# Foxhead-Studio/InsTaG

Measured on AMD Instinct MI355X. Metric: train-step frames/sec @512x512, 100k Gaussians, higher is better.
Workload: dtype f32; 1 GPU; C3: train_face step, 100k Gaussians + 6 grid encodes + UMF/PMF motion nets (DeepSpeech feats), 512x512, SH degree 1, image + attention map in one raster pass, L1+DSSIM, Adam; targets = uniform noise (SURVEY 8d); gaussians=100000, sh_degree=1, parallelism=dp1, ranks_reported_by_backend=1, execution=hipGraph replay, timing=one window of 1714 steps after 5 warm-up steps

## Files before the change

### instag_amd/csrc/common.hpp

```cpp
#pragma once
#include <hip/hip_runtime.h>
#include <stdint.h>
#include <stddef.h>
#include <algorithm>
#include <mutex>
#include <set>
#include <string>
#include <utility>

#include "instag_hip.h"

namespace instag {

void set_error(const std::string& msg);

#define INSTAG_CHECK_HIP(expr)                                                                  \
  do {                                                                                          \
    hipError_t _e = (expr);                                                                     \
    if (_e != hipSuccess) {                                                                     \
      ::instag::set_error(std::string(#expr) + ": " + hipGetErrorString(_e));                   \
      return INSTAG_E_HIP;                                                                      \
    }                                                                                           \
  } while (0)

#define INSTAG_REQUIRE(cond, msg)                                                               \
  do {                                                                                          \
    if (!(cond)) {                                                                              \
      ::instag::set_error(std::string(msg));                                                    \
      return INSTAG_E_ARG;                                                                      \
    }                                                                                           \
  } while (0)

#define INSTAG_CHECK_LAUNCH() INSTAG_CHECK_HIP(hipGetLastError())

#define INSTAG_TRY(expr) do { if (int rc_ = (expr)) return rc_; } while (0)

enum ProfKernel {
  K_PREPROCESS = 0, K_DUPLICATE = 1, K_SORT = 2, K_RANGES = 3, K_BLEND_FWD = 4, K_BLEND_BWD = 5,
  K_PREPROCESS_BWD = 6, K_GRID_FWD = 7, K_GRID_BWD = 8, K_SH_FWD = 9, K_SH_BWD = 10,
  K_MLP_FWD = 11, K_MLP_BWD = 12, K_MLP_WGRAD = 13, K_LOSS_FWD = 14, K_LOSS_BWD = 15, K_BLEND_BWD_MEAN = 16,
  K_EMPTY_BRACKET = 17,
};
struct ProfScope {
  ProfScope(int kernel, hipStream_t stream);
  ~ProfScope();
  int kernel_;
  hipStream_t stream_;
  hipEvent_t start_ = nullptr;
  int graph_slot_ = -1;
};

template <typename T>
static inline T div_up(T a, T b) { return (a + b - 1) / b; }

static inline int set_max_dynamic_lds(const void* kernel, int bytes) {
  static std::mutex mu;
  static std::set<std::pair<const void*, int>> done;
  int dev = 0;
  INSTAG_CHECK_HIP(hipGetDevice(&dev));
  std::lock_guard<std::mutex> lk(mu);
  if (done.count({kernel, dev})) return INSTAG_OK;
  INSTAG_CHECK_HIP(hipFuncSetAttribute(kernel, hipFuncAttributeMaxDynamicSharedMemorySize, bytes));
  done.insert({kernel, dev});
  return INSTAG_OK;
}

static inline size_t align_up(size_t v, size_t a) { return (v + a - 1) / a * a; }

struct Arena {
  size_t off = 0;
  size_t take(size_t n) { const size_t o = off; off += align_up(n, 64); return o; }
};

constexpr int TILE_X = 16;
constexpr int TILE_Y = 16;
constexpr int REC_FLOATS = 16;

enum RecSlot { R_X = 0, R_Y, R_CA, R_CB, R_CC, R_OP, R_R, R_G, R_B, R_DEPTH, R_NX, R_NY, R_NZ, R_EXTRA,
               R_OFFSET, R_RECT };

struct GeomLayout {
  size_t rec2d, cov3d, tiles_touched, point_offsets, flags, cull_thr;
  size_t depth_key, depth_key_alt, order_a, order;
  size_t dsort_zero, dsort_zero_words;
  size_t dsort_digit_base;
  size_t dsort_partials;
  size_t scan_state, scan_state_words;
  size_t tile_partials, tile_total, tile_dropped, pre_zero_words;
  uint32_t pre_blocks;
  uint32_t dsort_blocks, dkey_blocks;
  size_t total;
};
GeomLayout geom_layout(int32_t N);

struct ImageLayout {
  size_t ranges, n_contrib, final_T;
  size_t tile_rounds;
  size_t blend_mode;
  size_t total;
};
ImageLayout image_layout(int32_t H, int32_t W);

struct BinningLayout {
  size_t keys_unsorted, vals_unsorted, keys, vals, ktmp, vtmp, gid_unsorted, point_list;
  size_t tsort_zero, tsort_zero_words;
  size_t tsort_digit_base;
  size_t tsort_partials;
  size_t sort_count;
  uint32_t tsort_blocks;
  size_t seg_state, seg_slots, seg_queue, seg_count, row_flag, row_flag_stride;
  size_t fwd_sync, seg_flag;
  size_t total;
};
constexpr int SEG_LEN = 128;
constexpr int SEG_FLOATS = 14;
constexpr int TILE_PIX = TILE_X * TILE_Y;
BinningLayout binning_layout(int64_t R, int32_t H, int32_t W);

}
```

### instag_amd/csrc/grid.hip

```cpp
#include <cstdlib>

#include "common.hpp"
#include "device_math.hpp"

namespace instag {
namespace {

constexpr int GRID_BLOCK = 256;
constexpr uint32_t LDS_BUDGET_FLOATS = 16384;

template <uint32_t D>
__device__ __forceinline__ uint32_t fast_hash(const uint32_t pos_grid[D]) {
  constexpr uint32_t primes[7] = {1u, 2654435761u, 805459861u, 3674653429u, 2097192037u, 1434869437u, 2165219737u};
  uint32_t result = 0;
#pragma unroll
  for (uint32_t i = 0; i < D; ++i) result ^= pos_grid[i] * primes[i];
  return result;
}

template <uint32_t D>
__device__ __forceinline__ uint32_t grid_index(uint32_t gridtype, bool align_corners, uint32_t hashmap_size,
                                               uint32_t resolution, const uint32_t pos_grid[D]) {
  uint32_t stride = 1, index = 0;
#pragma unroll
// ... 453 lines not shown

inline bool dc_supported(uint32_t D, uint32_t C) { return D >= 2 && D <= 5 && (C == 1 || C == 2 || C == 4 || C == 8); }

#define DISPATCH_DC(D, C, FN, ...)                                                            \
  switch (D) {                                                                                \
    case 2: switch (C) { case 1: return FN<2, 1>(__VA_ARGS__); case 2: return FN<2, 2>(__VA_ARGS__); \
                         case 4: return FN<2, 4>(__VA_ARGS__); case 8: return FN<2, 8>(__VA_ARGS__); } break; \
    case 3: switch (C) { case 1: return FN<3, 1>(__VA_ARGS__); case 2: return FN<3, 2>(__VA_ARGS__); \
                         case 4: return FN<3, 4>(__VA_ARGS__); case 8: return FN<3, 8>(__VA_ARGS__); } break; \
    case 4: switch (C) { case 1: return FN<4, 1>(__VA_ARGS__); case 2: return FN<4, 2>(__VA_ARGS__); \
                         case 4: return FN<4, 4>(__VA_ARGS__); case 8: return FN<4, 8>(__VA_ARGS__); } break; \
    case 5: switch (C) { case 1: return FN<5, 1>(__VA_ARGS__); case 2: return FN<5, 2>(__VA_ARGS__); \
                         case 4: return FN<5, 4>(__VA_ARGS__); case 8: return FN<5, 8>(__VA_ARGS__); } break; \
  }

}
}

using namespace instag;

extern "C" {

int instag_grid_encode_forward(const float* inputs, const float* embeddings, const int32_t* offsets, float* outputs,
                               uint32_t B, uint32_t D, uint32_t C, uint32_t L, float S, uint32_t H, float* dy_dx,
                               uint32_t gridtype, int align_corners, uint32_t interp, instag_stream_t stream) {
  INSTAG_REQUIRE(L >= 1 && L <= 64, "GridEncoding: L must be in [1,64]");
  INSTAG_REQUIRE(dc_supported(D, C), "GridEncoding: D must be 2..5 and C must be 1, 2, 4, or 8.");
  if (B == 0) return INSTAG_OK;
  INSTAG_REQUIRE(inputs && embeddings && offsets && outputs, "grid_encode_forward: NULL tensor");
  hipStream_t s = (hipStream_t)stream;
  DISPATCH_DC(D, C, run_forward, inputs, embeddings, offsets, outputs, B, L, S, H, dy_dx, gridtype,
              align_corners != 0, interp, s);
  set_error("GridEncoding: D must be 2..5 and C must be 1, 2, 4, or 8.");
  return INSTAG_E_ARG;
}

int instag_grid_encode_backward(const float* grad, const float* inputs, const float* embeddings,
                                const int32_t* offsets, float* grad_embeddings, uint32_t B, uint32_t D, uint32_t C,
                                uint32_t L, float S, uint32_t H, const float* dy_dx, float* grad_inputs,
                                uint32_t gridtype, int align_corners, uint32_t interp, instag_stream_t stream) {
  (void)embeddings;
  INSTAG_REQUIRE(L >= 1 && L <= 64, "GridEncoding: L must be in [1,64]");
  INSTAG_REQUIRE(dc_supported(D, C), "GridEncoding: D must be 2..5 and C must be 1, 2, 4, or 8.");
  if (B == 0) return INSTAG_OK;
  INSTAG_REQUIRE(grad && inputs && offsets && grad_embeddings, "grid_encode_backward: NULL tensor");
  hipStream_t s = (hipStream_t)stream;
  DISPATCH_DC(D, C, run_backward, grad, inputs, offsets, grad_embeddings, B, L, S, H, dy_dx, grad_inputs,
              gridtype, align_corners != 0, interp, s);
  set_error("GridEncoding: D must be 2..5 and C must be 1, 2, 4, or 8.");
  return INSTAG_E_ARG;
}

size_t instag_grid_total_variation_workspace_bytes(uint32_t total_params, uint32_t C) {
  return align_up((size_t)total_params * sizeof(uint32_t), 256) + (size_t)total_params * C * sizeof(unsigned long long);
}

int instag_grid_total_variation(const float* inputs, const float* embeddings, float* grad, const int32_t* offsets,
                                float weight, uint32_t B, uint32_t D, uint32_t C, uint32_t L, float S, uint32_t H,
                                uint32_t gridtype, int align_corners, uint32_t total_params, void* workspace,
                                size_t workspace_bytes, instag_stream_t stream) {
  INSTAG_REQUIRE(L >= 1 && L <= 64, "GridEncoding: L must be in [1,64]");
  INSTAG_REQUIRE(dc_supported(D, C), "GridEncoding: D must be 2..5 and C must be 1, 2, 4, or 8.");
  if (B == 0) return INSTAG_OK;
  INSTAG_REQUIRE(inputs && embeddings && grad && offsets, "grad_total_variation: NULL tensor");
  const size_t need = instag_grid_total_variation_workspace_bytes(total_params, C);
  if (workspace == nullptr || workspace_bytes < need) { set_error("grad_total_variation: workspace too small"); return INSTAG_E_SPACE; }
  hipStream_t s = (hipStream_t)stream;
  INSTAG_CHECK_HIP(hipMemsetAsync(workspace, 0, need, s));
  uint32_t* counts = (uint32_t*)workspace;
  unsigned long long* acc = (unsigned long long*)((char*)workspace + align_up((size_t)total_params * sizeof(uint32_t), 256));
  DISPATCH_DC(D, C, run_tv, inputs, embeddings, grad, offsets, weight, B, L, S, H, gridtype, align_corners != 0, counts,
              acc, s);
  set_error("GridEncoding: D must be 2..5 and C must be 1, 2, 4, or 8.");
  return INSTAG_E_ARG;
}

}

namespace instag {
namespace {

constexpr uint32_t TP_MAX_L = 16;
inline bool tp_fits_lds(uint32_t total_params) { return (size_t)12 * total_params <= 156 * 1024; }

struct TriPlaneArgs {
  const float* xyz;
  const float* tables[3];
  const int32_t* offsets;
  uint32_t N, L, H;
  float S, bound;
  const float* shift;
  uint32_t shift_stride;
  float shift_scale;
};

__device__ __forceinline__ void tp_point(const TriPlaneArgs& a, uint32_t b, float p[3]) {
#pragma unroll
  for (int k = 0; k < 3; ++k) p[k] = a.xyz[3 * b + k];
  if (a.shift) {
#pragma unroll
    for (int k = 0; k < 3; ++k) p[k] += a.shift_scale * a.shift[(size_t)b * a.shift_stride + k];
  }
}

__device__ __forceinline__ void plane_coords(int plane, const float p[3], float x[2]) {
  x[0] = plane == 1 ? p[1] : p[0];
  x[1] = plane == 0 ? p[1] : p[2];
}

struct TpLevel { float scale; uint32_t stride, offset; };

__device__ __forceinline__ void tp_levels(const TriPlaneArgs& a, TpLevel* s_lv) {
  if (threadIdx.x < a.L) {
    const LevelGeom lg = level_geom(a.offsets, threadIdx.x, a.S, a.H);
    s_lv[threadIdx.x] = TpLevel{lg.scale, lg.resolution + 1, (uint32_t)a.offsets[threadIdx.x]};
  }
}

template <int THREADS, bool ZERO_ACC>
__device__ __forceinline__ void tp_stage_table(float* __restrict__ s_tab, float* __restrict__ s_acc,
                                               const float* __restrict__ tab, uint32_t T) {
  if ((T & 3u) == 0 && (reinterpret_cast<uintptr_t>(tab) & 15) == 0) {
    const float4* src = reinterpret_cast<const float4*>(tab);
    float4* dst = reinterpret_cast<float4*>(s_tab);
    float4* acc = reinterpret_cast<float4*>(s_acc);
    const uint32_t n4 = T >> 2;
#pragma unroll 8
    for (uint32_t i = threadIdx.x; i < n4; i += THREADS) {
      dst[i] = src[i];
      if (ZERO_ACC) acc[i] = make_float4(0.f, 0.f, 0.f, 0.f);
    }
  } else {
#pragma unroll 8
    for (uint32_t i = threadIdx.x; i < T; i += THREADS) {
      s_tab[i] = tab[i];
      if (ZERO_ACC) s_acc[i] = 0.f;
    }
  }
}

__global__ void __launch_bounds__(GRID_BLOCK)
triplane_forward_kernel(TriPlaneArgs a, float* __restrict__ out ) {
  extern __shared__ __align__(16) float s_tab[];
  __shared__ TpLevel s_lv[TP_MAX_L];
  const uint32_t per_block = (a.N + gridDim.x - 1) / gridDim.x;
  const uint32_t b0 = blockIdx.x * per_block, b1 = min(a.N, b0 + per_block);
  const uint32_t T = (uint32_t)a.offsets[a.L];
  const float inv2b = 1.0f / (2.0f * a.bound);
  tp_levels(a, s_lv);
  for (int plane = 0; plane < 3; ++plane) {
    __syncthreads();
    tp_stage_table<GRID_BLOCK, false>(s_tab, nullptr, a.tables[plane], T);
    __syncthreads();
    for (uint32_t b = b0 + threadIdx.x; b < b1; b += GRID_BLOCK) {
      float p[3];
      tp_point(a, b, p);
      float xw[2];
      plane_coords(plane, p, xw);
      const float x0 = (xw[0] + a.bound) * inv2b, x1 = (xw[1] + a.bound) * inv2b;
      const bool oob = x0 < 0.f || x0 > 1.f || x1 < 0.f || x1 > 1.f;
      float* o = out + (size_t)b * 3 * a.L + plane * a.L;
#pragma unroll 4
      for (uint32_t l = 0; l < a.L; ++l) {
        float v = 0.f;
        if (!oob) {
          const TpLevel lv = s_lv[l];
// ... 637 lines not shown
```

### instag_amd/csrc/mlp.hip

```cpp
#include <cstdlib>

#include "common.hpp"

namespace instag {
namespace {

using f32x16 = __attribute__((ext_vector_type(16))) float;
constexpr int MLP_BLOCK = 256;

__device__ __forceinline__ constexpr int feat(int r, int h) { return (r & 3) + 8 * (r >> 2) + 4 * h; }

template <int KC = 0>
__device__ __forceinline__ void load_block(const float* __restrict__ X, size_t row, bool valid, int Krt, int b, int h,
                                           f32x16& v) {
  const int K = KC > 0 ? KC : Krt;
  const float* __restrict__ base = X + (valid ? row * (size_t)K : 0);
  if ((K & 3) == 0) {
#pragma unroll
    for (int q = 0; q < 4; ++q) {
      const int f0 = 32 * b + 8 * q + 4 * h;
      const bool ok = valid && f0 < K;
      const float4 t = *reinterpret_cast<const float4*>(base + (ok ? f0 : 0));
      v[4 * q + 0] = ok ? t.x : 0.f; v[4 * q + 1] = ok ? t.y : 0.f;
      v[4 * q + 2] = ok ? t.z : 0.f; v[4 * q + 3] = ok ? t.w : 0.f;
// ... 239 lines not shown
            }
          }
          raw[b][4 * q] = t.x; raw[b][4 * q + 1] = t.y; raw[b][4 * q + 2] = t.z; raw[b][4 * q + 3] = t.w;
        }
    } else {
#pragma unroll
      for (int b = 0; b < KB0; ++b) load_block(X, row, valid, d.K0, b, h, raw[b]);
    }
  };
  int tile = blockIdx.x * 4 + wave;
  if (tile < ntiles) fetch(tile);
  for (; tile < ntiles; tile += tstride) {
    const size_t row = (size_t)tile * 32 + l31;
    const bool valid = row < (size_t)d.N;
    f32x16 in0[KB0];
#pragma unroll
    for (int b = 0; b < KB0; ++b) in0[b] = raw[b];
    if (tile + tstride < ntiles) fetch(tile + tstride);
    if (GLUE) {
      constexpr int K0 = GLUE_KX + GLUE_KA + GLUE_KE;
      float sa = 0.f, se = 0.f;
#pragma unroll
      for (int b = 0; b < KB0; ++b)
#pragma unroll
        for (int q = 0; q < 4; ++q) {
          const int f0 = 32 * b + 8 * q + 4 * h;
          float v[4] = {in0[b][4 * q], in0[b][4 * q + 1], in0[b][4 * q + 2], in0[b][4 * q + 3]};
          if (f0 >= GLUE_KX && f0 + 4 <= GLUE_KX + GLUE_KA) {
            sa += (v[0] * v[0] + v[1] * v[1]) + (v[2] * v[2] + v[3] * v[3]);
#pragma unroll
            for (int i = 0; i < 4; ++i) v[i] *= mul[b][4 * q + i];
          } else if (f0 >= GLUE_KX + GLUE_KA && f0 < K0) {
#pragma unroll
            for (int i = 0; i < 4; ++i)
              if (f0 + i < K0) {
                const float act = fmaxf(v[i], 0.f);
                se += act * act;
                v[i] = mul[b][4 * q + i] * act;
              }
          }
          if (valid && f0 < K0 && gf.h_in != nullptr) {
            float* hp = gf.h_in + row * K0 + f0;
            *reinterpret_cast<float2*>(hp) = make_float2(v[0], v[1]);
            if (f0 + 2 < K0) *reinterpret_cast<float2*>(hp + 2) = make_float2(v[2], v[3]);
          }
          in0[b][4 * q] = v[0]; in0[b][4 * q + 1] = v[1]; in0[b][4 * q + 2] = v[2]; in0[b][4 * q + 3] = v[3];
        }
      sa += __shfl_xor(sa, 32);
      se += __shfl_xor(se, 32);
      if (valid && h == 0) { gf.amb[3 * row] = sqrtf(sa); gf.amb[3 * row + 1] = sqrtf(se); gf.amb[3 * row + 2] = 0.f; }
    }
    f32x16 h1[HB];
    layer_forward<KQ0, KB0, HB>(w1, in0, h1, l31, h);
    relu_blocks<HB>(h1);
    if (A1) {
      store_blocks<HB, 8 * HQ>(A1, row, valid, d.H, h, h1);
    }
    f32x16 out[1];
    if (NL == 3) {
      f32x16 h2[HB];
      uint32_t sw1 = 0, sw2 = 0;
      layer_forward<HQ, HB, HB, KEEP>(w2, h1, h2, l31, h, &sw1);
      if constexpr (KEEP) S1[(size_t)tile * 64 + lane] = sw1;
      relu_blocks<HB>(h2);
      if (A2) {
        store_blocks<HB, 8 * HQ>(A2, row, valid, d.H, h, h2);
      }
      layer_forward<HQ, HB, 1, KEEP>(w3, h2, out, l31, h, &sw2);
      if constexpr (KEEP) S2[(size_t)tile * 64 + lane] = sw2;
    } else {
      uint32_t sw1 = 0;
      layer_forward<HQ, HB, 1, KEEP>(w2, h1, out, l31, h, &sw1);
      if constexpr (KEEP) S1[(size_t)tile * 64 + lane] = sw1;
    }
    store_block(Y, row, valid, d.O, 0, h, out[0]);
  }
}

struct GlueBwd {
  const float* aud; const float* eye_pre; const float* enc_a; const float* enc_e; const float* amb; const float* d_amb;
  float* d_enc_x; float* d_aud; float* d_eye; float* col_partials;
};

template <int KQ0, int HQ, int OQ, int NL, bool GLUE = false>
__global__ void __launch_bounds__(MLP_BLOCK) __attribute__((amdgpu_waves_per_eu(2)))
mlp_backward_kernel(MlpDims d, const float* __restrict__ dY, const uint32_t* __restrict__ S1,
                    const uint32_t* __restrict__ S2, const float* __restrict__ W1, const float* __restrict__ W2,
                    const float* __restrict__ W3, float* __restrict__ dZ1, float* __restrict__ dZ2,
                    float* dX, const float* dXadd ,
                    GlueBwd gl = GlueBwd{}) {
  extern __shared__ __align__(16) float s_w[];
  __shared__ float s_col[GLUE ? 4 : 1][GLUE ? 40 : 1];
  constexpr int KBG = (KQ0 + 3) / 4;
  float part[GLUE ? KBG : 1][4][4];
  if (GLUE) {
#pragma unroll
    for (int b = 0; b < KBG; ++b)
#pragma unroll
      for (int q = 0; q < 4; ++q)
#pragma unroll
        for (int i = 0; i < 4; ++i) part[b][q][i] = 0.f;
  }
  constexpr int KB0 = (KQ0 + 3) / 4, HB = (HQ + 3) / 4;
  constexpr int KP0 = KB0 * 32, HP = HB * 32;
  float* w1 = s_w;
  float* w2 = w1 + HP * (KP0 + 1);
  float* w3 = w2 + (NL == 3 ? HP : 32) * (HP + 1);
  if (dX || GLUE) stage_weights<HP, KB0>(w1, W1, d.H, d.K0);
  stage_weights<(NL == 3 ? HP : 32), HB>(w2, W2, NL == 3 ? d.H : d.O, d.H);
  if (NL == 3) stage_weights<32, HB>(w3, W3, d.O, d.H);
  __syncthreads();
  const int lane = threadIdx.x & 63, wave = threadIdx.x >> 6, l31 = lane & 31, h = lane >> 5;
  const int ntiles = (d.N + 31) / 32;
  const int tstride = gridDim.x * 4;
  f32x16 ndy;
  uint32_t ns1 = 0, ns2 = 0;
  auto fetch = [&](int tile) {
    const size_t row = (size_t)tile * 32 + l31;
    const bool valid = row < (size_t)d.N;
    load_block(dY, row, valid, d.O, 0, h, ndy);
    if constexpr (NL == 3) ns2 = S2[(size_t)tile * 64 + lane];
    ns1 = S1[(size_t)tile * 64 + lane];
  };
  int tile = blockIdx.x * 4 + wave;
  if (tile < ntiles) fetch(tile);
  for (; tile < ntiles; tile += tstride) {
    const size_t row = (size_t)tile * 32 + l31;
    const bool valid = row < (size_t)d.N;
    f32x16 dy[1];
    dy[0] = ndy;
    const uint32_t s1 = ns1, s2 = ns2;
    if (tile + tstride < ntiles) fetch(tile + tstride);
    f32x16 g1[HB];
    if constexpr (NL == 3) {
      f32x16 g2[HB];
      layer_backward<OQ, 1, HB>(w3, dy, g2, l31, h);
      mask_blocks<HB>(g2, s2);
      store_blocks<HB, 8 * HQ>(dZ2, row, valid, d.H, h, g2);
      layer_backward<HQ, HB, HB>(w2, g2, g1, l31, h);
    } else {
      layer_backward<OQ, 1, HB>(w2, dy, g1, l31, h);
    }
    mask_blocks<HB>(g1, s1);
    store_blocks<HB, 8 * HQ>(dZ1, row, valid, d.H, h, g1);
    if (GLUE) {
      f32x16 gx[KB0];
      layer_backward<HQ, HB, KB0>(w1, g1, gx, l31, h);
      if (valid) {
        const float na = gl.amb[3 * row], ne = gl.amb[3 * row + 1];
        const float ga = (gl.d_amb && na > 0.f) ? gl.d_amb[3 * row] / na : 0.f;
        const float ge = (gl.d_amb && ne > 0.f) ? gl.d_amb[3 * row + 1] / ne : 0.f;
#pragma unroll
        for (int b = 0; b < KB0; ++b)
#pragma unroll
          for (int q = 0; q < 4; ++q) {
            const int f0 = 32 * b + 8 * q + 4 * h;
            const float gw[4] = {gx[b][4 * q], gx[b][4 * q + 1], gx[b][4 * q + 2], gx[b][4 * q + 3]};
            if (f0 + 4 <= GLUE_KX) {
              *reinterpret_cast<float4*>(gl.d_enc_x + row * GLUE_KX + f0) = make_float4(gw[0], gw[1], gw[2], gw[3]);
            } else if (f0 >= GLUE_KX && f0 + 4 <= GLUE_KX + GLUE_KA) {
              const int k = f0 - GLUE_KX;
              const float4 a = *reinterpret_cast<const float4*>(gl.aud + row * GLUE_KA + k);
              const float4 ea = *reinterpret_cast<const float4*>(gl.enc_a + k);
              *reinterpret_cast<float4*>(gl.d_aud + row * GLUE_KA + k) =
                  make_float4(ea.x * gw[0] + ga * a.x, ea.y * gw[1] + ga * a.y, ea.z * gw[2] + ga * a.z,
                              ea.w * gw[3] + ga * a.w);
              part[b][q][0] += gw[0] * a.x; part[b][q][1] += gw[1] * a.y;
              part[b][q][2] += gw[2] * a.z; part[b][q][3] += gw[3] * a.w;
            } else if (f0 >= GLUE_KX + GLUE_KA && f0 < GLUE_KX + GLUE_KA + GLUE_KE) {
              const int k = f0 - GLUE_KX - GLUE_KA;
#pragma unroll
              for (int i = 0; i < 4; ++i) {
                if (k + i < GLUE_KE) {
                  const float pre = gl.eye_pre[row * GLUE_KE + k + i];
                  const float act = fmaxf(pre, 0.f);
                  gl.d_eye[row * GLUE_KE + k + i] = pre > 0.f ? (gl.enc_e[k + i] * gw[i] + ge * act) : 0.f;
                  part[b][q][i] += gw[i] * act;
                }
              }
            }
          }
      }
    } else if (dX) {
      f32x16 gx[KB0];
      layer_backward<HQ, HB, KB0>(w1, g1, gx, l31, h);
      if (dXadd) {
#pragma unroll
        for (int b = 0; b < KB0; ++b) {
          f32x16 prev;
          load_block(dXadd, row, valid, d.K0, b, h, prev);
          gx[b] += prev;
        }
      }
#pragma unroll
      for (int b = 0; b < KB0; ++b) store_block(dX, row, valid, d.K0, b, h, gx[b]);
    }
  }
  if (GLUE) {
    for (int i = threadIdx.x; i < 4 * 40; i += MLP_BLOCK) (&s_col[0][0])[i] = 0.f;
    __syncthreads();
#pragma unroll
    for (int b = 0; b < KBG; ++b)
#pragma unroll
      for (int q = 0; q < 4; ++q) {
        const int f0 = 32 * b + 8 * q + 4 * h;
        if (f0 >= GLUE_KX && f0 < GLUE_KX + GLUE_KA + GLUE_KE) {
#pragma unroll
          for (int i = 0; i < 4; ++i) {
            float v = part[b][q][i];
#pragma unroll
            for (int o = 16; o > 0; o >>= 1) v += __shfl_xor(v, o);
            if (l31 == 0 && f0 + i < GLUE_KX + GLUE_KA + GLUE_KE) s_col[wave][f0 + i - GLUE_KX] = v;
          }
        }
      }
    __syncthreads();
    if ((int)threadIdx.x < GLUE_KA + GLUE_KE)
      gl.col_partials[(size_t)blockIdx.x * (GLUE_KA + GLUE_KE) + threadIdx.x] =
          ((s_col[0][threadIdx.x] + s_col[1][threadIdx.x]) + s_col[2][threadIdx.x]) + s_col[3][threadIdx.x];
  }
}


struct Mlp2Dims { int N, K0, HA, OA, HB, OB; };

template <int KQ0, int HQA, int HQB>
size_t mlp2_lds_bytes() {
  constexpr int KP0 = (KQ0 + 3) / 4 * 32, HPA = (HQA + 3) / 4 * 32, HPB = (HQB + 3) / 4 * 32;
  return sizeof(float) * (HPA * (KP0 + 1) + 32 * (HPA + 1) + HPB * (KP0 + 1) + 32 * (HPB + 1));
}

template <int KQ0, int HQA, int OQA, int HQB, int OQB, bool KEEP >
__global__ void __launch_bounds__(MLP_BLOCK)
mlp2_forward_kernel(Mlp2Dims d, const float* __restrict__ X, const float* __restrict__ WA1,
                    const float* __restrict__ WA2, const float* __restrict__ WB1, const float* __restrict__ WB2,
                    float* __restrict__ YA, float* __restrict__ YB, float* __restrict__ A1A, float* __restrict__ A1B,
                    uint32_t* __restrict__ S1) {
  extern __shared__ __align__(16) float s_w[];
  constexpr int KB0 = (KQ0 + 3) / 4, HBA = (HQA + 3) / 4, HBB = (HQB + 3) / 4;
  constexpr int KP0 = KB0 * 32, HPA = HBA * 32, HPB = HBB * 32;
  static_assert(HBA == 1 && HBB == 1, "mlp2: the two heads' sign bits share one word per lane");
  float* wa1 = s_w;
  float* wa2 = wa1 + HPA * (KP0 + 1);
  float* wb1 = wa2 + 32 * (HPA + 1);
  float* wb2 = wb1 + HPB * (KP0 + 1);
  stage_weights<HPA, KB0>(wa1, WA1, d.HA, d.K0);
  stage_weights<32, HBA>(wa2, WA2, d.OA, d.HA);
  stage_weights<HPB, KB0>(wb1, WB1, d.HB, d.K0);
  stage_weights<32, HBB>(wb2, WB2, d.OB, d.HB);
  __syncthreads();
  const int lane = threadIdx.x & 63, wave = threadIdx.x >> 6, l31 = lane & 31, h = lane >> 5;
  const int ntiles = (d.N + 31) / 32;
  for (int tile = blockIdx.x * 4 + wave; tile < ntiles; tile += gridDim.x * 4) {
    const size_t row = (size_t)tile * 32 + l31;
    const bool valid = row < (size_t)d.N;
    f32x16 in0[KB0];
#pragma unroll
    for (int b = 0; b < KB0; ++b) load_block(X, row, valid, d.K0, b, h, in0[b]);
    uint32_t sw = 0;
    {
      f32x16 h1[HBA], out[1];
      layer_forward<KQ0, KB0, HBA>(wa1, in0, h1, l31, h);
      relu_blocks<HBA>(h1);
      if (A1A) store_blocks<HBA, 8 * HQA>(A1A, row, valid, d.HA, h, h1);
      layer_forward<HQA, HBA, 1, KEEP>(wa2, h1, out, l31, h, &sw);
      store_block(YA, row, valid, d.OA, 0, h, out[0]);
    }
    {
      f32x16 h1[HBB], out[1];
      layer_forward<KQ0, KB0, HBB>(wb1, in0, h1, l31, h);
      relu_blocks<HBB>(h1);
      if (A1B) store_blocks<HBB, 8 * HQB>(A1B, row, valid, d.HB, h, h1);
      layer_forward<HQB, HBB, 1, KEEP, 16>(wb2, h1, out, l31, h, &sw);
      store_block(YB, row, valid, d.OB, 0, h, out[0]);
    }
    if constexpr (KEEP) S1[(size_t)tile * 64 + lane] = sw;
  }
}

template <int KQ0, int HQA, int OQA, int HQB, int OQB>
__global__ void __launch_bounds__(MLP_BLOCK)
mlp2_backward_kernel(Mlp2Dims d, const float* __restrict__ dYA, const float* __restrict__ dYB,
                     const uint32_t* S1A, const uint32_t* S1B , const float* __restrict__ WA1,
                     const float* __restrict__ WA2, const float* __restrict__ WB1, const float* __restrict__ WB2,
                     float* __restrict__ dZ1A, float* __restrict__ dZ1B, float* dX,
                     const float* dXadd ) {
  extern __shared__ __align__(16) float s_w[];
  constexpr int KB0 = (KQ0 + 3) / 4, HBA = (HQA + 3) / 4, HBB = (HQB + 3) / 4;
  constexpr int KP0 = KB0 * 32, HPA = HBA * 32, HPB = HBB * 32;
  static_assert(HBA == 1 && HBB == 1, "mlp2: the two heads' sign bits share one word per lane");
  float* wa1 = s_w;
  float* wa2 = wa1 + HPA * (KP0 + 1);
  float* wb1 = wa2 + 32 * (HPA + 1);
  float* wb2 = wb1 + HPB * (KP0 + 1);
  if (dX) { stage_weights<HPA, KB0>(wa1, WA1, d.HA, d.K0); stage_weights<HPB, KB0>(wb1, WB1, d.HB, d.K0); }
  stage_weights<32, HBA>(wa2, WA2, d.OA, d.HA);
  stage_weights<32, HBB>(wb2, WB2, d.OB, d.HB);
  __syncthreads();
  const int lane = threadIdx.x & 63, wave = threadIdx.x >> 6, l31 = lane & 31, h = lane >> 5;
  const int ntiles = (d.N + 31) / 32;
  const int tstride = gridDim.x * 4;
  f32x16 ndya, ndyb;
  uint32_t nsa = 0, nsb = 0;
// ... 29 lines not shown
    }
    {
      f32x16 g1[HBB], gb[KB0];
      layer_backward<OQB, 1, HBB>(wb2, dyb, g1, l31, h);
      mask_blocks<HBB, 16>(g1, sb);
      store_blocks<HBB, 8 * HQB>(dZ1B, row, valid, d.HB, h, g1);
      if (dX) {
        layer_backward<HQB, HBB, KB0>(wb1, g1, gb, l31, h);
#pragma unroll
        for (int b = 0; b < KB0; ++b) gx[b] += gb[b];
      }
    }
    if (dX) {
      if (dXadd) {
#pragma unroll
        for (int b = 0; b < KB0; ++b) {
          f32x16 prev;
          load_block(dXadd, row, valid, d.K0, b, h, prev);
          gx[b] += prev;
        }
      }
#pragma unroll
      for (int b = 0; b < KB0; ++b) store_block(dX, row, valid, d.K0, b, h, gx[b]);
    }
  }
}

struct WgVirt {
  int job;
  const float *xb, *xc, *mb, *mc;
  int Ka, Kb, Kc, pad;
};

template <int OB, int KB, bool VIRT = false>
__device__ __forceinline__ void weight_grad_body(const float* __restrict__ dZ, const float* __restrict__ In, int N, int O,
                                                 int K, float* __restrict__ partial, float* s_acc, int block,
                                                 int nblocks, const WgVirt* virt = nullptr) {
  constexpr int TILES = OB * KB;
  constexpr int TW = TILES >= 4 ? 4 : TILES;
  constexpr int RS = 4 / TW;
  constexpr int MYT = (TILES + TW - 1) / TW;
  const int lane = threadIdx.x & 63, wave = threadIdx.x >> 6, l31 = lane & 31, h = lane >> 5;
  const int tw = wave % TW, rs = wave / TW;
  const bool busy = wave < TW * RS;
  const int per_block = (((N + nblocks - 1) / nblocks) + 1) & ~1;
  const long b0 = (long)block * per_block, b1 = min((long)N, b0 + per_block);
  const int per_split = ((((int)max(0l, b1 - b0) + RS - 1) / RS) + 1) & ~1;
  const long w0 = b0 + (long)rs * per_split;
  const long w1 = busy ? min(b1, w0 + per_split) : w0;
  int tt[MYT], tb[MYT];
  bool live[MYT], oin[MYT], kin[MYT];
#pragma unroll
  for (int j = 0; j < MYT; ++j) {
    const int idx = tw + j * TW;
    live[j] = idx < TILES;
    tt[j] = live[j] ? idx / KB : 0;
    tb[j] = live[j] ? idx % KB : 0;
    oin[j] = live[j] && 32 * tt[j] + l31 < O;
    kin[j] = live[j] && 32 * tb[j] + l31 < K;
  }
  const float* bp[MYT];
  int bs[MYT];
  float bm[MYT];
  bool brelu[MYT];
#pragma unroll
  for (int j = 0; j < MYT; ++j) {
    const int col = 32 * tb[j] + l31;
    bp[j] = In + col; bs[j] = K; bm[j] = 1.f; brelu[j] = false;
    if (VIRT && kin[j]) {
      if (col < virt->Ka) { bp[j] = In + col; bs[j] = virt->Ka; }
      else if (col < virt->Ka + virt->Kb) {
        bp[j] = virt->xb + (col - virt->Ka); bs[j] = virt->Kb; bm[j] = virt->mb[col - virt->Ka];
      } else {
        const int c2 = col - virt->Ka - virt->Kb;
        bp[j] = virt->xc + c2; bs[j] = virt->Kc; bm[j] = virt->mc[c2]; brelu[j] = true;
      }
    }
  }
  f32x16 acc[MYT];
#pragma unroll
  for (int j = 0; j < MYT; ++j)
#pragma unroll
    for (int i = 0; i < 16; ++i) acc[j][i] = 0.f;
  constexpr int UNROLL = 6;
  for (long r0 = w0; r0 < w1; r0 += 2 * UNROLL) {
    float a[UNROLL][MYT], bb[UNROLL][MYT];
#pragma unroll
    for (int u = 0; u < UNROLL; ++u) {
      const long row = r0 + 2 * u + h;
      const bool ok = row < w1;
#pragma unroll
      for (int j = 0; j < MYT; ++j) {
        a[u][j] = (ok && oin[j]) ? dZ[row * O + 32 * tt[j] + l31] : 0.f;
        float v = (ok && kin[j]) ? bp[j][row * bs[j]] : 0.f;
        if (VIRT) {
          v = brelu[j] ? fmaxf(v, 0.f) : v;
          v *= bm[j];
        }
        bb[u][j] = v;
      }
    }
#pragma unroll
    for (int u = 0; u < UNROLL; ++u)
#pragma unroll
      for (int j = 0; j < MYT; ++j)
        acc[j] = __builtin_amdgcn_mfma_f32_32x32x2f32(a[u][j], bb[u][j], acc[j], 0, 0, 0);
  }
  float* dst = partial + (size_t)block * O * K;
  if (RS == 1) {
#pragma unroll
    for (int j = 0; j < MYT; ++j) {
      if (!live[j] || !busy) continue;
#pragma unroll
      for (int i = 0; i < 16; ++i) {
        const int o = 32 * tt[j] + feat(i, h), k = 32 * tb[j] + l31;
        if (o < O && k < K) dst[o * K + k] = acc[j][i];
      }
    }
    return;
  }
  for (int r = 0; r < RS; ++r) {
    if (busy && rs == r) {
#pragma unroll
      for (int i = 0; i < 16; ++i) {
        float* p = &s_acc[(tw * 16 + i) * 64 + lane];
        *p = (r == 0) ? acc[0][i] : (*p + acc[0][i]);
      }
    }
    __syncthreads();
  }
  for (int idx = threadIdx.x; idx < TILES * 1024; idx += MLP_BLOCK) {
    const int ln = idx & 63, i = (idx >> 6) & 15, tile = idx >> 10;
    const int t = tile / KB, b = tile - t * KB;
    const int o = 32 * t + feat(i, ln >> 5), k = 32 * b + (ln & 31);
    if (o < O && k < K) dst[o * K + k] = s_acc[idx];
  }
}

constexpr int WG_MAX_JOBS = 16;
struct WgJob { const float* dz; const float* in; float* partial; float* dw; int N, O, K, pad; };
struct WgBatch { WgJob j[WG_MAX_JOBS]; WgVirt virt; };

constexpr int WG_WAVES = 4;
__global__ void __launch_bounds__(MLP_BLOCK) __attribute__((amdgpu_waves_per_eu(WG_WAVES)))
weight_grad_batched_kernel(WgBatch b) {
  __shared__ float s_acc[3 * 1024];
  const WgJob job = b.j[blockIdx.y];
  const int ob = (job.O + 31) / 32, kb = (job.K + 31) / 32;
  if ((int)blockIdx.y == b.virt.job) {
    if (ob == 1) weight_grad_body<1, 3, true>(job.dz, job.in, job.N, job.O, job.K, job.partial, s_acc, blockIdx.x, gridDim.x, &b.virt);
    else weight_grad_body<2, 3, true>(job.dz, job.in, job.N, job.O, job.K, job.partial, s_acc, blockIdx.x, gridDim.x, &b.virt);
    return;
  }
  if (ob == 1 && kb == 1) weight_grad_body<1, 1>(job.dz, job.in, job.N, job.O, job.K, job.partial, s_acc, blockIdx.x, gridDim.x);
  else if (ob == 1 && kb == 2) weight_grad_body<1, 2>(job.dz, job.in, job.N, job.O, job.K, job.partial, s_acc, blockIdx.x, gridDim.x);
  else if (ob == 1 && kb == 3) weight_grad_body<1, 3>(job.dz, job.in, job.N, job.O, job.K, job.partial, s_acc, blockIdx.x, gridDim.x);
  else if (ob == 2 && kb == 1) weight_grad_body<2, 1>(job.dz, job.in, job.N, job.O, job.K, job.partial, s_acc, blockIdx.x, gridDim.x);
  else if (ob == 2 && kb == 2) weight_grad_body<2, 2>(job.dz, job.in, job.N, job.O, job.K, job.partial, s_acc, blockIdx.x, gridDim.x);
  else weight_grad_body<2, 3>(job.dz, job.in, job.N, job.O, job.K, job.partial, s_acc, blockIdx.x, gridDim.x);
}

__global__ void __launch_bounds__(256)
weight_grad_reduce_batched_kernel(WgBatch b, int nparts) {
  __shared__ float s_part[4][64];
  const WgJob job = b.j[blockIdx.y];
  const int count = job.O * job.K;
  if ((int)blockIdx.x * 64 >= count) return;
  const int e = threadIdx.x & 63, g = threadIdx.x >> 6;
  const int i = blockIdx.x * 64 + e;
  float s = 0.f;
  if (i < count) {
    const int per = (nparts + 3) / 4;
    const int p0 = g * per, p1 = min(nparts, p0 + per);
#pragma unroll 8
    for (int p = p0; p < p1; ++p) s += job.partial[(size_t)p * count + i];
  }
  s_part[g][e] = s;
  __syncthreads();
  if (g == 0 && i < count) job.dw[i] = ((s_part[0][e] + s_part[1][e]) + s_part[2][e]) + s_part[3][e];
}

inline int wg_blocks(int N) { return std::max(1, std::min(256, (N + 255) / 256)); }

inline int mlp_blocks(int ntiles) {
  return std::max(1, std::min(512, (ntiles + 3) / 4));
}

template <int KB0, int HB, int NL>
size_t mlp_lds_bytes() {
  constexpr int KP0 = KB0 * 32, HP = HB * 32;
  return sizeof(float) * (HP * (KP0 + 1) + (NL == 3 ? HP : 32) * (HP + 1) + (NL == 3 ? 32 * (HP + 1) : 0));
}

template <int KQ0, int HQ, int OQ, int NL>
int run_fwd(const MlpDims& d, const float* x, const float* w1, const float* w2, const float* w3, float* y, float* a1,
            float* a2, uint32_t* s1, uint32_t* s2, hipStream_t s) {
  const int ntiles = (d.N + 31) / 32;
  const int blocks = mlp_blocks(ntiles);
  ProfScope p(K_MLP_FWD, s);
  const size_t lds = mlp_lds_bytes<(KQ0 + 3) / 4, (HQ + 3) / 4, NL>();
  if (s1) mlp_forward_kernel<KQ0, HQ, OQ, NL, false, true><<<blocks, MLP_BLOCK, lds, s>>>(d, x, w1, w2, w3, y, a1, a2, s1, s2);
  else mlp_forward_kernel<KQ0, HQ, OQ, NL, false, false><<<blocks, MLP_BLOCK, lds, s>>>(d, x, w1, w2, w3, y, a1, a2, s1, s2);
  INSTAG_CHECK_LAUNCH();
  return INSTAG_OK;
}
template <int KQ0, int HQ, int OQ, int NL>
int run_bwd(const MlpDims& d, const float* dy, const uint32_t* s1, const uint32_t* s2, const float* w1, const float* w2,
            const float* w3, float* dz1, float* dz2, float* dx, const float* dx_add, hipStream_t s) {
  const int ntiles = (d.N + 31) / 32;
  const int blocks = mlp_blocks(ntiles);
  ProfScope p(K_MLP_BWD, s);
  mlp_backward_kernel<KQ0, HQ, OQ, NL><<<blocks, MLP_BLOCK, mlp_lds_bytes<(KQ0 + 3) / 4, (HQ + 3) / 4, NL>(), s>>>(
      d, dy, s1, s2, w1, w2, w3, dz1, dz2, dx, dx_add);
  INSTAG_CHECK_LAUNCH();
  return INSTAG_OK;
}

#define MLP_DISPATCH(FN, ...)                                                                      \
  do {                                                                                             \
    const int kq = (d.K0 + 7) / 8, hq = (d.H + 7) / 8, oq = (d.O + 7) / 8;                          \
    if (NL == 3) {                                                                                 \
      if (kq == 10 && hq == 8 && oq == 2) return FN<10, 8, 2, 3>(__VA_ARGS__);                      \
      if (kq == 10 && hq == 4 && oq == 2) return FN<10, 4, 2, 3>(__VA_ARGS__);                      \
      if (kq == 10 && hq == 2 && oq == 1) return FN<10, 2, 1, 3>(__VA_ARGS__);                      \
    } else {                                                                                       \
      if (kq == 5 && hq == 4 && oq == 4) return FN<5, 4, 4, 2>(__VA_ARGS__);                        \
      if (kq == 5 && hq == 4 && oq == 1) return FN<5, 4, 1, 2>(__VA_ARGS__);                        \
      if (kq == 5 && hq == 2 && oq == 1) return FN<5, 2, 1, 2>(__VA_ARGS__);                        \
    }                                                                                              \
    const int kb = (d.K0 + 31) / 32, hb = (d.H + 31) / 32;                                           \
    if (NL == 2) {                                                                                 \
      if (kb == 1 && hb == 1) return FN<4, 4, 4, 2>(__VA_ARGS__);                                   \
      if (kb == 2 && hb == 1) return FN<8, 4, 4, 2>(__VA_ARGS__);                                   \
      if (kb == 3 && hb == 1) return FN<12, 4, 4, 2>(__VA_ARGS__);                                  \
      if (kb == 1 && hb == 2) return FN<4, 8, 4, 2>(__VA_ARGS__);                                   \
      if (kb == 2 && hb == 2) return FN<8, 8, 4, 2>(__VA_ARGS__);                                   \
      if (kb == 3 && hb == 2) return FN<12, 8, 4, 2>(__VA_ARGS__);                                  \
    } else {                                                                                       \
      if (kb == 1 && hb == 1) return FN<4, 4, 4, 3>(__VA_ARGS__);                                   \
      if (kb == 2 && hb == 1) return FN<8, 4, 4, 3>(__VA_ARGS__);                                   \
      if (kb == 3 && hb == 1) return FN<12, 4, 4, 3>(__VA_ARGS__);                                  \
      if (kb == 1 && hb == 2) return FN<4, 8, 4, 3>(__VA_ARGS__);                                   \
      if (kb == 2 && hb == 2) return FN<8, 8, 4, 3>(__VA_ARGS__);                                   \
      if (kb == 3 && hb == 2) return FN<12, 8, 4, 3>(__VA_ARGS__);                                  \
    }                                                                                              \
  } while (0)

int check_dims(int N, int K0, int H, int O, int NL) {
  INSTAG_REQUIRE(N >= 0, "mlp: N must be >= 0");
  INSTAG_REQUIRE(NL == 2 || NL == 3, "mlp: only 2- or 3-layer MLPs are supported");
  INSTAG_REQUIRE(K0 >= 1 && K0 <= 96, "mlp: input width must be in [1,96]");
  INSTAG_REQUIRE(H >= 1 && H <= 64, "mlp: hidden width must be in [1,64]");
  INSTAG_REQUIRE(O >= 1 && O <= 32, "mlp: output width must be in [1,32]");
  return INSTAG_OK;
}

}
}

using namespace instag;

extern "C" {

int instag_mlp_forward(const float* x, const float* w1, const float* w2, const float* w3, float* y, float* a1,
                       float* a2, uint32_t* s1, uint32_t* s2, int32_t N, int32_t K0, int32_t H, int32_t O, int32_t NL,
                       instag_stream_t stream) {
  if (int e = check_dims(N, K0, H, O, NL)) return e;
  INSTAG_REQUIRE(x && w1 && w2 && y && (NL == 2 || w3), "mlp_forward: NULL tensor");
  INSTAG_REQUIRE(NL == 2 || (s1 == nullptr) == (s2 == nullptr), "mlp_forward: s1 and s2 go together");
  if (N == 0) return INSTAG_OK;
  const MlpDims d{N, K0, H, O};
  hipStream_t s = (hipStream_t)stream;
  MLP_DISPATCH(run_fwd, d, x, w1, w2, w3, y, a1, a2, s1, s2, s);
  set_error("mlp_forward: unsupported shape");
  return INSTAG_E_ARG;
}

int instag_mlp_backward_add(const float* dy, const uint32_t* s1, const uint32_t* s2, const float* w1, const float* w2,
                            const float* w3, float* dz1, float* dz2, float* dx, const float* dx_add, int32_t N,
                            int32_t K0, int32_t H, int32_t O, int32_t NL, instag_stream_t stream) {
  if (int e = check_dims(N, K0, H, O, NL)) return e;
  INSTAG_REQUIRE(dy && s1 && w1 && w2 && dz1 && (NL == 2 || (w3 && s2 && dz2)), "mlp_backward: NULL tensor");
  INSTAG_REQUIRE(dx_add == nullptr || dx != nullptr, "mlp_backward: dx_add needs dx");
  if (N == 0) return INSTAG_OK;
  const MlpDims d{N, K0, H, O};
  hipStream_t s = (hipStream_t)stream;
  MLP_DISPATCH(run_bwd, d, dy, s1, s2, w1, w2, w3, dz1, dz2, dx, dx_add, s);
  set_error("mlp_backward: unsupported shape");
  return INSTAG_E_ARG;
}

int instag_mlp_backward(const float* dy, const uint32_t* s1, const uint32_t* s2, const float* w1, const float* w2,
                        const float* w3, float* dz1, float* dz2, float* dx, int32_t N, int32_t K0, int32_t H,
                        int32_t O, int32_t NL, instag_stream_t stream) {
  return instag_mlp_backward_add(dy, s1, s2, w1, w2, w3, dz1, dz2, dx, nullptr, N, K0, H, O, NL, stream);
}
// ... 166 lines not shown
```

Before: 1057 frames/s.

## Rebalance register/LDS budgets so weight-grad, MLP backward and tri-plane backward co-reside

```diff
diff --git a/instag_amd/csrc/common.hpp b/instag_amd/csrc/common.hpp
--- a/instag_amd/csrc/common.hpp
+++ b/instag_amd/csrc/common.hpp
@@ -67,6 +67,15 @@
 
 static inline size_t align_up(size_t v, size_t a) { return (v + a - 1) / a * a; }
 
+constexpr int SIMD_VGPRS = 512;
+constexpr int CU_LDS_BYTES = 160 * 1024;
+constexpr int WG_PER_CU = 2;
+constexpr int WG_VGPRS_MIN = 176;
+constexpr int WG_VGPRS_MAX = 192;
+constexpr int WG_LDS_BYTES = 2 * 1024 * 4;
+static_assert(WG_PER_CU * WG_VGPRS_MAX <= SIMD_VGPRS && (WG_PER_CU + 1) * WG_VGPRS_MIN > SIMD_VGPRS,
+              "the weight-gradient launch's register allocation must cap it at WG_PER_CU waves per SIMD");
+
 struct Arena {
   size_t off = 0;
   size_t take(size_t n) { const size_t o = off; off += align_up(n, 64); return o; }
diff --git a/instag_amd/csrc/grid.hip b/instag_amd/csrc/grid.hip
--- a/instag_amd/csrc/grid.hip
+++ b/instag_amd/csrc/grid.hip
@@ -559,6 +559,14 @@
 
 constexpr uint32_t TP_MAX_L = 16;
 inline bool tp_fits_lds(uint32_t total_params) { return (size_t)12 * total_params <= 156 * 1024; }
+
+constexpr uint32_t TP_BWD_STATIC_LDS = 256;
+constexpr uint32_t TP_BWD_WAVE_VGPRS = 108;
+constexpr uint32_t TP_MOTION_PARAMS = 9464;
+static_assert((size_t)12 * TP_MOTION_PARAMS + TP_BWD_STATIC_LDS + WG_PER_CU * WG_LDS_BYTES <= (size_t)CU_LDS_BYTES,
+              "a motion field's tri-plane backward must fit a CU's LDS beside two weight-gradient workgroups");
+static_assert((WG_PER_CU - 1) * WG_VGPRS_MAX + 2 * TP_BWD_WAVE_VGPRS <= SIMD_VGPRS,
+              "a tri-plane backward workgroup must fit a SIMD beside one weight-gradient wave");
 
 struct TriPlaneArgs {
   const float* xyz;
diff --git a/instag_amd/csrc/mlp.hip b/instag_amd/csrc/mlp.hip
--- a/instag_amd/csrc/mlp.hip
+++ b/instag_amd/csrc/mlp.hip
@@ -345,13 +345,13 @@
   float* d_enc_x; float* d_aud; float* d_eye; float* col_partials;
 };
 
-template <int KQ0, int HQ, int OQ, int NL, bool GLUE = false>
-__global__ void __launch_bounds__(MLP_BLOCK) __attribute__((amdgpu_waves_per_eu(2)))
-mlp_backward_kernel(MlpDims d, const float* __restrict__ dY, const uint32_t* __restrict__ S1,
-                    const uint32_t* __restrict__ S2, const float* __restrict__ W1, const float* __restrict__ W2,
-                    const float* __restrict__ W3, float* __restrict__ dZ1, float* __restrict__ dZ2,
-                    float* dX, const float* dXadd ,
-                    GlueBwd gl = GlueBwd{}) {
+template <int KQ0, int HQ, int OQ, int NL, bool GLUE>
+__device__ __forceinline__ void mlp_backward_body(const MlpDims& d, const float* __restrict__ dY,
+                                                  const uint32_t* __restrict__ S1, const uint32_t* __restrict__ S2,
+                                                  const float* __restrict__ W1, const float* __restrict__ W2,
+                                                  const float* __restrict__ W3, float* __restrict__ dZ1,
+                                                  float* __restrict__ dZ2, float* dX, const float* dXadd,
+                                                  const GlueBwd& gl) {
   extern __shared__ __align__(16) float s_w[];
   __shared__ float s_col[GLUE ? 4 : 1][GLUE ? 40 : 1];
   constexpr int KBG = (KQ0 + 3) / 4;
@@ -482,6 +482,29 @@
       gl.col_partials[(size_t)blockIdx.x * (GLUE_KA + GLUE_KE) + threadIdx.x] =
           ((s_col[0][threadIdx.x] + s_col[1][threadIdx.x]) + s_col[2][threadIdx.x]) + s_col[3][threadIdx.x];
   }
+}
+
+template <int KQ0, int HQ, int OQ, int NL, bool GLUE = false>
+__global__ void __launch_bounds__(MLP_BLOCK) __attribute__((amdgpu_waves_per_eu(2)))
+mlp_backward_kernel(MlpDims d, const float* __restrict__ dY, const uint32_t* __restrict__ S1,
+                    const uint32_t* __restrict__ S2, const float* __restrict__ W1, const float* __restrict__ W2,
+                    const float* __restrict__ W3, float* __restrict__ dZ1, float* __restrict__ dZ2,
+                    float* dX, const float* dXadd ,
+                    GlueBwd gl = GlueBwd{}) {
+  mlp_backward_body<KQ0, HQ, OQ, NL, GLUE>(d, dY, S1, S2, W1, W2, W3, dZ1, dZ2, dX, dXadd, gl);
+}
+
+constexpr int MLP_LEAN_WAVES = 4;
+static_assert(WG_PER_CU * WG_VGPRS_MAX + SIMD_VGPRS / MLP_LEAN_WAVES <= SIMD_VGPRS,
+              "a wave of mlp_backward_lean_kernel must fit a SIMD that is full of weight-gradient waves");
+template <int KQ0, int HQ, int OQ>
+__global__ void __launch_bounds__(MLP_BLOCK) __attribute__((amdgpu_waves_per_eu(MLP_LEAN_WAVES)))
+mlp_backward_lean_kernel(MlpDims d, const float* __restrict__ dY, const uint32_t* __restrict__ S1,
+                         const float* __restrict__ W1, const float* __restrict__ W2, float* __restrict__ dZ1,
+                         float* dX, const float* dXadd ) {
+  static_assert((HQ + 3) / 4 == 1 && (KQ0 + 3) / 4 <= 2 && OQ == 1,
+                "mlp_backward_lean_kernel: one hidden block, at most two input blocks, at most 8 outputs");
+  mlp_backward_body<KQ0, HQ, OQ, 2, false>(d, dY, S1, nullptr, W1, W2, nullptr, dZ1, nullptr, dX, dXadd, GlueBwd{});
 }
 
 
@@ -677,7 +700,7 @@
   for (int j = 0; j < MYT; ++j)
 #pragma unroll
     for (int i = 0; i < 16; ++i) acc[j][i] = 0.f;
-  constexpr int UNROLL = 6;
+  constexpr int UNROLL = 10;
   for (long r0 = w0; r0 < w1; r0 += 2 * UNROLL) {
     float a[UNROLL][MYT], bb[UNROLL][MYT];
 #pragma unroll
@@ -714,6 +737,8 @@
     }
     return;
   }
+  static_assert(RS == 1 || TILES * 1024 * sizeof(float) <= WG_LDS_BYTES,
+                "weight_grad_body: the combine holds at most two tiles");
   for (int r = 0; r < RS; ++r) {
     if (busy && rs == r) {
 #pragma unroll
@@ -736,10 +761,12 @@
 struct WgJob { const float* dz; const float* in; float* partial; float* dw; int N, O, K, pad; };
 struct WgBatch { WgJob j[WG_MAX_JOBS]; WgVirt virt; };
 
-constexpr int WG_WAVES = 4;
-__global__ void __launch_bounds__(MLP_BLOCK) __attribute__((amdgpu_waves_per_eu(WG_WAVES)))
+constexpr int WG_WAVES = 2;
+constexpr int WG_ACC_FLOATS = WG_LDS_BYTES / sizeof(float);
+__global__ void __launch_bounds__(MLP_BLOCK)
+__attribute__((amdgpu_waves_per_eu(WG_WAVES, WG_WAVES), amdgpu_num_vgpr(WG_VGPRS_MAX / 2)))
 weight_grad_batched_kernel(WgBatch b) {
-  __shared__ float s_acc[3 * 1024];
+  __shared__ float s_acc[WG_ACC_FLOATS];
   const WgJob job = b.j[blockIdx.y];
   const int ob = (job.O + 31) / 32, kb = (job.K + 31) / 32;
   if ((int)blockIdx.y == b.virt.job) {
@@ -805,8 +832,13 @@
   const int ntiles = (d.N + 31) / 32;
   const int blocks = mlp_blocks(ntiles);
   ProfScope p(K_MLP_BWD, s);
-  mlp_backward_kernel<KQ0, HQ, OQ, NL><<<blocks, MLP_BLOCK, mlp_lds_bytes<(KQ0 + 3) / 4, (HQ + 3) / 4, NL>(), s>>>(
-      d, dy, s1, s2, w1, w2, w3, dz1, dz2, dx, dx_add);
+  constexpr int KB0 = (KQ0 + 3) / 4, HB = (HQ + 3) / 4;
+  if constexpr (NL == 2 && HB == 1 && KB0 <= 2 && OQ == 1)
+    mlp_backward_lean_kernel<KQ0, HQ, OQ><<<blocks, MLP_BLOCK, mlp_lds_bytes<KB0, HB, NL>(), s>>>(d, dy, s1, w1, w2, dz1,
+                                                                                                 dx, dx_add);
+  else
+    mlp_backward_kernel<KQ0, HQ, OQ, NL><<<blocks, MLP_BLOCK, mlp_lds_bytes<KB0, HB, NL>(), s>>>(
+        d, dy, s1, s2, w1, w2, w3, dz1, dz2, dx, dx_add);
   INSTAG_CHECK_LAUNCH();
   return INSTAG_OK;
 }
```

Result: slower. 1041 frames/s (-1.5%).
